# jc-bao/gym-formation

Hardware: AMD Instinct MI355X
Metric: env-steps/sec (higher is better)
Workload: dtype f32

## Files before the change

gym-formation_amd/csrc/fg_common.hpp:

```cpp
#ifndef FG_COMMON_HPP_
#define FG_COMMON_HPP_


#include <hip/hip_runtime.h>
#include <stdint.h>
#include <stdio.h>
#include <string.h>

#include "formation_hip.h"


namespace fg {

#define FG_DEV __device__ __forceinline__
constexpr int FG_PRODUCER_PRIO = 2;
typedef float f32x4 __attribute__((ext_vector_type(4)));
typedef float f32x2 __attribute__((ext_vector_type(2)));

#ifndef FG_F64
#define FG_F64 0
#endif
#if FG_F64
typedef double real;
typedef double2 real2;
// ... 11 lines not shown
FG_DEV float rabs(float a) { return fabsf(a); }
FG_DEV float rsqrt_(float a) { return sqrtf(a); }
FG_DEV float rfma(float a, float b, float c) { return __builtin_fmaf(a, b, c); }
FG_DEV float hw_sqrt(float a) { return __builtin_amdgcn_sqrtf(a); }
FG_DEV float hw_rcp(float a) { return __builtin_amdgcn_rcpf(a); }
FG_DEV float hw_log(float a) { return __logf(a); }
FG_DEV float hw_exp(float a) { return __expf(a); }
FG_DEV double rmin(double a, double b) { return fmin(a, b); }
FG_DEV double rmax(double a, double b) { return fmax(a, b); }
FG_DEV double rabs(double a) { return fabs(a); }
FG_DEV double rsqrt_(double a) { return sqrt(a); }
FG_DEV double rfma(double a, double b, double c) { return __builtin_fma(a, b, c); }
FG_DEV double hw_sqrt(double a) { return sqrt(a); }
FG_DEV double hw_rcp(double a) { return 1.0 / a; }
FG_DEV double hw_log(double a) { return log(a); }
FG_DEV double hw_exp(double a) { return exp(a); }

#if FG_F64
struct KWall {
    int32_t vertical, soft;
    double axis_pos, end0, end1, width;
};
struct KParams {
    double dt, damping, contact_force, contact_margin, sensitivity, mass, dist_min, collide_thresh;
    int32_t world_length, auto_reset;
    uint64_t seed, rng_offset;
    double accel, max_speed, u_noise;
    int32_t num_walls;
    KWall walls[FG_MAX_WALLS];
    int32_t obs_env_pitch, env_index_base;
    const uint64_t* rng_offset_dev;
    const double* agent_props;
    const double* comm_state;
    int32_t obs_placed, reserved0;
};
#else
typedef FgParams KParams;
typedef FgWall KWall;
#endif
FG_DEV uint64_t rng_base(const KParams& p) { return p.rng_offset + (p.rng_offset_dev ? *p.rng_offset_dev : 0ull); }

__host__ __device__ constexpr int npad(int n) { return (n + 3) & ~3; }
__host__ __device__ constexpr int env_block_floats(int n) { return 10 * n + 6 * npad(n); }
FG_DEV real2* env_tables(real2* smem, int ee, int n) {
    return reinterpret_cast<real2*>(reinterpret_cast<real*>(smem) + ee * env_block_floats(n));
}
FG_DEV const real2* env_tables(const real2* smem, int ee, int n) {
    return reinterpret_cast<const real2*>(reinterpret_cast<const real*>(smem) + ee * env_block_floats(n));
}
__host__ __device__ constexpr int step_lds_bytes(int n, int e, bool opts) {
    return (e * env_block_floats(n) + 72 + (opts ? 3 * npad(n) + 2 * e * n : 0)) * (int)sizeof(real);
}
constexpr real FAR_AWAY = 1.0e18f;

constexpr int FG_POLICY_MAX_LEVELS = 10;
struct FgPolicyLevels {
    int per, L;
    float inv_per;
    float inv_sub[FG_POLICY_MAX_LEVELS];
};

struct Args {
    KParams p;
    int B, N, K, obs_every;
    real inv_n;
    int do_phys, do_post;
    int groups;
// ... 167 lines not shown
```

gym-formation_amd/csrc/fg_obs_writers.hpp:

```cpp
#ifndef FG_OBS_WRITERS_HPP_
#define FG_OBS_WRITERS_HPP_

#include "fg_common.hpp"

namespace fg {

template <class V2> FG_DEV V2 lds_if(bool c, const V2* __restrict__ p, int idx_if_true) {
    V2 t = p[c ? idx_if_true : 0];
    t.x = c ? t.x : 0.0f; t.y = c ? t.y : 0.0f;
    return t;
}

constexpr bool FG_ROWS_MERGED = true;
template <int NC, int NW, int E, int PACE = 0>
FG_DEV void write_obs_rows(const real2* __restrict__ tables0, int env_stride, int w,
                           real2* __restrict__ out_env0, size_t env_units, int El, int parts,
                           int wg_part = 0, int wg_parts = 1, bool pace_on = true) {
    constexpr int N = NC;
    constexpr int WPE = (E >= NW) ? 1 : NW / E;
    constexpr int ESTEP = (E >= NW) ? NW : 1;
    static_assert((E >= NW) ? (E % NW == 0) : (NW % E == 0), "waves and envs must tile");
    const int lane = threadIdx.x & 63;
    const int row0 = (E >= NW) ? 0 : w % WPE;
    constexpr unsigned ROWU = 3u * N;
// ... 85 lines not shown
            for (int c = 0; c < CD; ++c) {
                const int u = lane + 64 * c;
                Pm[c] = lds_if(u >= 1 && u < N, AA, u - 1);
                Pu[c] = lds_if(u >= 1 && u < N, AA, u);
            }
#pragma unroll
            for (int c = 0; c < CS; ++c) sv[c] = lds_if(lane + 64 * c < 2 * N, AA, N + lane + 64 * c);
            const int nshare = WPE * wg_parts, share = wg_part * WPE + row0;
            const int PER = (N + nshare - 1) / nshare;
            const int r_end = min(N, (share + 1) * PER);
#pragma unroll 2
            for (int r = share * PER; r < r_end; ++r) {
                const real2 xp = AA[r];
                const real2 x0 = AA[(lane == 0 ? 4 * N : 0) + r];
                real2* __restrict__ orow = out + (unsigned)r * ROWU;
#pragma unroll
                for (int c = 0; c < CD; ++c) {
                    const int u = lane + 64 * c;
                    const real2 x = (c == 0) ? x0 : xp;
                    const real2 cc = (u - 1 >= r) ? Pu[c] : Pm[c];
                    if ((parts & 1) && u < N) orow[u] = make_real2(cc.x - x.x, cc.y - x.y);
                }
#pragma unroll
                for (int c = 0; c < CS; ++c)
                    if ((parts & 2) && lane + 64 * c < 2 * N) orow[N + lane + 64 * c] = sv[c];
                if (PACE > 0 && pace_on) __builtin_amdgcn_s_sleep(PACE);
            }
        }
    }
}

template <int NC, int RT> constexpr int tile_units() { return (3 * NC * RT + 16 + 2 + 1) & ~1; }

template <int NC, int NW, int E, int RT, bool STREAM>
FG_DEV void write_obs_tiled(const float2* __restrict__ tables0, int env_stride, int w, float2* __restrict__ tiles,
                            float2* __restrict__ out_env0, size_t unit0, size_t env_units, int El) {
    constexpr int N = NC;
    constexpr int WPE = (E >= NW) ? 1 : NW / E;
    static_assert((E >= NW) ? (E % NW == 0) : (NW % E == 0), "waves and envs must tile");
    static_assert(N <= 32 && N % RT == 0, "tiled writer: N <= 32, RT divides N");
    constexpr unsigned ROWU = 3u * N, TU = ROWU * RT;
    constexpr int TILES_ENV = N / RT;
    constexpr int MY_TILES = (TILES_ENV + WPE - 1) / WPE;
    const int lane = threadIdx.x & 63;
    float2* tile0 = tiles + w * 2 * tile_units<NC, RT>();
    constexpr int RW = 64 / N;
    const int rsub = lane / N, u = lane - rsub * N;
    const bool act = rsub < RW;
    const int xoff = (u == 0) ? 4 * N : 0;
    constexpr int RS = 64 / (2 * N);
    const int ssub = lane / (2 * N), sidx = lane - ssub * 2 * N;
    const int e_first = (E >= NW) ? w : w / WPE, e_step = (E >= NW) ? NW : E;
    const int t_first = (E >= NW) ? 0 : w % WPE;
    const int n_env = (El > e_first) ? (El - e_first + e_step - 1) / e_step : 0;
    const int total = n_env * MY_TILES;

    constexpr unsigned ENVU = ROWU * N;
    const unsigned pad = (unsigned)(env_units - ENVU);
    static_assert(!STREAM || (E >= NW && NC >= 16), "streaming form: waves own whole envs, rows of >= 16 units");
    const bool own = STREAM && ((unit0 & 15) == 0) && (pad == 0 || (pad < 16 && (env_units & 15) == 0));
    auto head_units = [&](int ee) -> unsigned {
        return (own && pad == 0) ? (16u - (unsigned)(((size_t)ee * env_units) & 15)) & 15u : 0u;
    };
    auto extra_units = [&](int ee) -> unsigned {
        if (!own) return 0u;
        if (pad) return pad;
        return (ee + 1 < El) ? head_units(ee + 1) : 0u;
    };

// ... 17 lines not shown
        }
        const unsigned par = (unsigned)((unit0 + (size_t)ee * env_units + (size_t)r0 * ROWU) & 1);
        float2* img = tile0 + (t & 1) * tile_units<NC, RT>() + par;
#pragma unroll
        for (int rb = 0; rb < RT; rb += RW) {
            const int rl = rb + rsub;
            if (act && rl < RT) {
                const int r = r0 + rl;
                const float2 x = AA[xoff + r];
                const float2 c = (u - 1 >= r) ? Pu : Pm;
                img[(unsigned)rl * ROWU + (unsigned)u] = make_float2(c.x - x.x, c.y - x.y);
            }
        }
#pragma unroll
        for (int rb = 0; rb < RT; rb += RS) {
            const int rl = rb + ssub;
            if (ssub < RS && rl < RT) img[(unsigned)rl * ROWU + (unsigned)(N + sidx)] = sv;
        }
        if (STREAM && r0 + RT == N) {
            const unsigned x = extra_units(ee);
            if ((unsigned)lane < x) {
                float2 val = make_float2(0.f, 0.f);
                if (pad == 0) {
                    static_assert(ROWU >= 16, "the line remainder must stay inside row 0 of the next env");
                    const float2* __restrict__ A1 = tables0 + (size_t)(ee + 1) * env_stride;
                    const float2 a = A1[lane == 0 ? 3 * N : lane], b = A1[0];
                    const bool rel = lane >= 1 && lane < N;
                    val = make_float2(a.x - (rel ? b.x : 0.f), a.y - (rel ? b.y : 0.f));
                }
                img[TU + (unsigned)lane] = val;
            }
        }
    };
    auto stream = [&](int t) {
        int ee, r0; locate(t, ee, r0);
        if (r0 >= N) return;
        const unsigned par = (unsigned)((unit0 + (size_t)ee * env_units + (size_t)r0 * ROWU) & 1);
        const float2* img = tile0 + (t & 1) * tile_units<NC, RT>() + par;
        float2* __restrict__ out = out_env0 + (size_t)ee * env_units + (size_t)r0 * ROWU;
        if constexpr (!STREAM) {
            if (par && lane == 0) out[0] = img[0];
            constexpr unsigned NPMAX = TU >> 1;
            const unsigned npair = (TU - par) >> 1;
            const f32x4* src4 = reinterpret_cast<const f32x4*>(img + par);
            f32x4* __restrict__ dst4 = reinterpret_cast<f32x4*>(out + par);
#pragma unroll
            for (unsigned q0 = 0; q0 < NPMAX; q0 += 64) {
                const unsigned q = q0 + lane;
                if (q < npair) dst4[q] = src4[q];
            }
            if (((TU - par) & 1u) && lane == 63) out[TU - 1] = img[TU - 1];
        } else {
            const unsigned s = (r0 == 0) ? head_units(ee) : 0u;
            const unsigned end = TU + ((r0 + RT == N) ? extra_units(ee) : 0u);
            const unsigned p2 = (par + s) & 1u;
            if (p2 && lane == 0) out[s] = img[s];
            constexpr unsigned NPMAX = (TU + 16) >> 1;
            const unsigned npair = (end - s - p2) >> 1;
            const f32x4* src4 = reinterpret_cast<const f32x4*>(img + s + p2);
            f32x4* __restrict__ dst4 = reinterpret_cast<f32x4*>(out + s + p2);
            constexpr unsigned NFULL = ((TU - 16) >> 1) / 64;
#pragma unroll
            for (unsigned c = 0; c < NFULL; ++c) {
                const f32x4 v = src4[c * 64 + lane];
                asm volatile("s_waitcnt lgkmcnt(0)" ::: "memory");
                dst4[c * 64 + lane] = v;
                asm volatile("" ::: "memory");
                __builtin_amdgcn_s_sleep(1);
            }
#pragma unroll
            for (unsigned q0 = NFULL * 64; q0 < NPMAX; q0 += 64) {
                const unsigned q = q0 + lane;
                if (q < npair) dst4[q] = src4[q];
            }
            if (((end - s - p2) & 1u) && lane == 63) out[end - 1] = img[end - 1];
        }
    };
    if (total > 0) compose(0);
    for (int t = 0; t < total; ++t) {
        if (t + 1 < total) compose(t + 1);
        stream(t);
    }
}

constexpr int FG_WR_GATHER = 64;
template <int NC> constexpr int gather_passes() { return (3 * NC * NC / 2 + 2 + 63) / 64; }
template <int NC> constexpr int gather_lut_units() { return 2 * gather_passes<NC>() * 64 * 2; }

template <int NC>
FG_DEV void build_gather_lut(uint4* __restrict__ lut, int t, int nthreads) {
    constexpr int N = NC, ROWU = 3 * N, TU = ROWU * N, P = gather_passes<NC>() * 64;
    static_assert(N >= 2 && 5 * N < 65536, "gather writer: table offsets are 16-bit, the table's zeros are the 0 operand");
    auto operands = [&](int unit, unsigned& a, unsigned& b) {
        const int r = unit / ROWU, u = unit - r * ROWU;
        if (u == 0) { a = N; b = 4 * N + r; }
        else if (u < N) { a = (u - 1 >= r) ? u : u - 1; b = r; }
        else { a = u; b = N; }
    };
    for (int e = t; e < 2 * P; e += nthreads) {
        const int par = e / P, q = e - par * P;
        const int npair = (TU - par) >> 1;
        const bool tail = ((TU - par) & 1) != 0;
        int unit = -1, kind = 0;
        if (q < npair) { unit = 2 * q + par; kind = 2; }
        else if (par && q == npair) { unit = 0; kind = 1; }
        else if (tail && q == npair + par) { unit = TU - 1; kind = 1; }
        unsigned a0 = N, b0 = N, a1 = N, b1 = N;
        if (kind >= 1) operands(unit, a0, b0);
        if (kind == 2) operands(unit + 1, a1, b1);
        lut[e] = make_uint4(a0 | (b0 << 16), a1 | (b1 << 16), (unsigned)(unit < 0 ? 0 : unit) | ((unsigned)kind << 16), 0u);
    }
}

template <int NC> struct GatherEntries {
// ... 203 lines not shown
```

gym-formation_amd/csrc/fg_rollout_kernels.hpp:

```cpp
#ifndef FG_ROLLOUT_KERNELS_HPP_
#define FG_ROLLOUT_KERNELS_HPP_

#include "fg_common.hpp"
#include "fg_pair_loops.hpp"
#include "fg_obs_writers.hpp"
#include "fg_policy_kernels.hpp"

namespace fg {

__host__ __device__ constexpr int roll_block_floats(int n) { return 20 * n + 6 * npad(n); }
template <int NC, int WR, int NWW, int E> constexpr int roll_writer_units() {
    if constexpr (WR == 0) return 0;
    else if constexpr (roll_writer_obs16(WR)) return 2 * NWW * obs16_tile_words<NC, NWW, E>() / 2;
    else if constexpr (WR == FG_WR_GATHER)
        return gather_lut_units<NC>() > E * 3 * NC * NC / 2 ? gather_lut_units<NC>() : E * 3 * NC * NC / 2;
    else return 2 * NWW * tile_units<NC, WR - 1>();
}

template <int NC, int TW, int E, int WR, int PER> constexpr int roll_lds_base_bytes() {
    return E * roll_block_floats(NC) * (int)sizeof(real) + roll_writer_units<NC, WR, TW / 64, E>() * (int)sizeof(float2) +
           (PER > 0 ? E * policy_block_units(NC) * (int)sizeof(float2) : 0);
}
template <int NC, int E> constexpr int roll_rew_floats() { return 2 * 3 * E * NC; }
template <int NC, int TW, int E, int WR, int PER> constexpr bool roll_rew_in_lds() {
// ... 203 lines not shown
                }
            }
            int slot = k;
            bool want_obs = a.obs != nullptr;
            if (a.obs_every > 1) { want_obs = want_obs && ((k + 1) % a.obs_every == 0); slot = k / a.obs_every; }
            if (want_obs) {
                const size_t unit0 = ((size_t)slot * a.B + b0) * (size_t)a.obs_pitch;
                const size_t env_units = (size_t)a.obs_pitch;
                const real2* tables0 = reinterpret_cast<const real2*>(smemf) + (k & 1) * 5 * N;
                if constexpr (WR == 0)
                    write_obs_rows<NC, NWW, E>(tables0, roll_block_floats(N) / 2, (tid - TP) >> 6,
                                               reinterpret_cast<real2*>(a.obs) + unit0, env_units, El, 3);
                else if constexpr (WR == FG_WR_GATHER) {
                  if (use_span)
                    Span::write(span_lut, tables0, (tid - TP) >> 6, reinterpret_cast<real2*>(a.obs) + unit0);
                  else {
                    GatherEntries<(WR == FG_WR_GATHER ? NC : 2)> gather_entries;
                    write_obs_gather<NC, NWW, E>(tables0, roll_block_floats(N) / 2, (tid - TP) >> 6,
                                                 reinterpret_cast<const uint4*>(smemf + E * roll_block_floats(N)),
                                                 reinterpret_cast<real2*>(a.obs) + unit0, unit0, env_units, El, gather_entries);
                  }
                }
#if !FG_F64
                else if constexpr (roll_writer_obs16(WR)) {
                    static_assert((E * roll_block_floats(NC)) % 4 == 0, "the 16-bit writer's tiles start on a 16-byte boundary");
                    write_obs16<NC, NWW, E, WR>(tables0, roll_block_floats(N) / 2, (tid - TP) >> 6,
                                                reinterpret_cast<uint32_t*>(smemf + E * roll_block_floats(N)),
                                                reinterpret_cast<uint32_t*>(a.obs) + unit0, unit0, El);
                }
#endif
                else
                    write_obs_tiled<NC, NWW, E, WR - 1, STREAM>(tables0, roll_block_floats(N) / 2, (tid - TP) >> 6,
                                                                reinterpret_cast<real2*>(smemf + E * roll_block_floats(N)),
                                                                reinterpret_cast<real2*>(a.obs) + unit0, unit0, env_units, El);
            }
        }
        __syncthreads();
    };
    if constexpr (ACT4) {
        for (int k = 0; k < a.K; k += 4) {
            if (producer && k + 4 < a.K) load_batch(nxt, k + 4);
            pipeline_step(k, cur[1], u_odd);
            if (k + 1 < a.K) pipeline_step(k + 1, cur[2], u_odd);
            if (k + 2 < a.K) pipeline_step(k + 2, cur[3], u_odd);
            if (k + 3 < a.K) pipeline_step(k + 3, nxt[0], u_odd);
#pragma unroll
            for (int t = 0; t < 4; ++t) cur[t] = nxt[t];
        }
    } else {
        for (int k = 0; k < a.K; k += 2) {
            pipeline_step(k, u_odd, u_even);
            if (k + 1 < a.K) pipeline_step(k + 1, u_even, u_odd);
        }
    }
    if (valid) {
        int is = i, bs = b;
        asm volatile("" : "+v"(is), "+v"(bs));
        const size_t so = (size_t)bs * N + is;
        a.px[so] = p.x; a.py[so] = p.y; a.vx[so] = v.x; a.vy[so] = v.y;
    }
    if (a.step && env_ok && i == 0) a.step[b] = t_step;
}

template <int NC, int A, int E, int TW, int PER = 0, bool BATCHES = false>
__global__ __launch_bounds__(E * 64 + TW) void rollout_kernel_wide(const Args a) {
    constexpr bool POLICY = PER > 0;
    static_assert(!(BATCHES && POLICY), "the batch-pipelined single step takes its actions from the caller");
// ... 300 lines not shown
```

gym-formation_amd/formation_gym/_native.py:

```python
import ctypes
import os
import subprocess

_HERE = os.path.dirname(os.path.abspath(__file__))
_PKG_ROOT = os.path.dirname(_HERE)
LIB_PATH = os.path.join(_PKG_ROOT, "lib", "libformation_hip.so")
BUILD_SCRIPT = os.path.join(_PKG_ROOT, "csrc", "build.sh")

ABI_VERSION = 8
MAX_WALLS = 4
AGENT_PROPS = 8
AGENT_IMMOVABLE, AGENT_NO_COLLIDE, AGENT_GHOST, AGENT_SCRIPTED = 1, 2, 4, 8

FG_OK = 0
FG_ERR_BAD_ARG = -1
FG_ERR_UNSUPPORTED_N = -2
FG_ERR_ALIGNMENT = -3
FG_ERR_HIP = -4


class FgWall(ctypes.Structure):
    _fields_ = [("vertical", ctypes.c_int32), ("axis_pos", ctypes.c_float), ("end0", ctypes.c_float),
                ("end1", ctypes.c_float), ("width", ctypes.c_float), ("soft", ctypes.c_int32)]


class FgParams(ctypes.Structure):
    _fields_ = [
        ("dt", ctypes.c_float),
        ("damping", ctypes.c_float),
        ("contact_force", ctypes.c_float),
        ("contact_margin", ctypes.c_float),
        ("sensitivity", ctypes.c_float),
        ("mass", ctypes.c_float),
        ("dist_min", ctypes.c_float),
        ("collide_thresh", ctypes.c_float),
        ("world_length", ctypes.c_int32),
        ("auto_reset", ctypes.c_int32),
        ("seed", ctypes.c_uint64),
        ("rng_offset", ctypes.c_uint64),
        ("accel", ctypes.c_float),
        ("max_speed", ctypes.c_float),
        ("u_noise", ctypes.c_float),
        ("num_walls", ctypes.c_int32),
        ("walls", FgWall * 4),
        ("obs_env_pitch", ctypes.c_int32),
        ("env_index_base", ctypes.c_int32),
        ("rng_offset_dev", ctypes.c_void_p),
        ("agent_props", ctypes.c_void_p),
        ("comm_state", ctypes.c_void_p),
        ("obs_placed", ctypes.c_int32),
        ("reserved0", ctypes.c_int32),
    ]


FG_SCN_BASIC, FG_SCN_PARTIAL, FG_SCN_RANGE, FG_SCN_OBSTACLE = 1, 2, 3, 4
FG_ACT_ONEHOT5, FG_ACT_INDEX, FG_ACT_ARGMAX = 1, 2, 3
FG_OBS_F16, FG_OBS_BF16 = 1, 2


def obs_format(dtype):
    import torch
    if dtype is None:
        return 0
    if dtype == torch.float16:
        return FG_OBS_F16
    if dtype == torch.bfloat16:
        return FG_OBS_BF16
    raise ValueError("obs_dtype must be None, torch.float16 or torch.bfloat16; got %r" % (dtype,))


class FgScenario(ctypes.Structure):
    _fields_ = [
        ("kind", ctypes.c_int32),
        ("num_landmarks", ctypes.c_int32),
        ("num_obstacles", ctypes.c_int32),
        ("num_obs", ctypes.c_int32),
        ("obs_range", ctypes.c_float),
        ("obstacle_size", ctypes.c_float),
        ("obstacle_vx", ctypes.c_float),
        ("obstacle_vy", ctypes.c_float),
        ("obstacle_floor", ctypes.c_float),
        ("penalty", ctypes.c_float),
        ("variant", ctypes.c_int32),
        ("reserved", ctypes.c_int32),
# ... 265 lines not shown
```

gym-formation_amd/formation_gym/environment.py:

```python
import numbers

import numpy as np
import torch

from . import _native, actor_rollout, spaces

cam_range = 2


class MultiAgentEnv(object):
    metadata = {'render.modes': ['human', 'rgb_array']}

    def __init__(self, world, reset_callback=None, reward_callback=None,
                 observation_callback=None, info_callback=None,
                 done_callback=None, post_step_callback=None,
                 shared_viewer=True, discrete_action=False):
        self.world = world
        self.world_length = self.world.world_length
        self.current_step = 0
        self.agents = self.world.policy_agents
        self.num_agents = len(world.policy_agents)
        self.reset_callback = reset_callback
        self.reward_callback = reward_callback
        self.observation_callback = observation_callback
        self.info_callback = info_callback
        self.done_callback = done_callback
        self.post_step_callback = post_step_callback
        self.num_envs = world.num_envs
        self.scenario = world.scenario
        if self.scenario is None:
            raise ValueError("world.scenario is not set: make_world() must attach the Scenario "
                             "that owns the batched kernels")
        self.discrete_action_space = bool(discrete_action)
        self.discrete_action_input = False
        self.force_discrete_action = bool(getattr(world, 'discrete_action', False))
        self.shared_reward = world.collaborative if hasattr(world, 'collaborative') else False
        self.time = 0
        self.auto_reset = False
# ... 137 lines not shown

    def _rollout_out(self, want, out, K, obs_every, policy, obs_dtype=None):
        placed = out is None and self.default_placed and obs_dtype is None
        if placed:
            out = self._default_out(K, obs_every, policy)
        elif out is None or out is False:
            return {k: self._fresh_out(k, want[k], obs_dtype) for k in want}, False
        own_buffers = True
        for k in ("log_prob", "rnn_states", "idx"):
            if k not in want:
                continue
            if placed and tuple(getattr(out.get(k), "shape", ())) != want[k]:
                out[k] = self._fresh_out(k, want[k])
            elif k not in out:
                out, own_buffers = dict(out, **{k: self._fresh_out(k, want[k])}), False
            elif k == "rnn_states":
                self._state_tensor("out['rnn_states']", out[k], want[k], None)
            elif k == "idx" and (not torch.is_tensor(out[k]) or out[k].dtype != torch.int32):
                raise ValueError("out['idx'] must be an int32 tensor of shape %s" % (want[k],))
        return out, own_buffers

    def _fresh_out(self, k, shape, obs_dtype=None):
        if k == "done":
            return torch.zeros(shape, dtype=torch.uint8, device=self._act.device)
        if k == "idx":
            return torch.empty(shape, dtype=torch.int32, device=self._act.device)
        return torch.empty(shape, dtype=(obs_dtype or torch.float32) if k == "obs" else torch.float32, device=self._act.device)

    def _run_rollout(self, lead_key, want, out, own_buffers, K, obs_every, obs_dtype, bind, unbound, args, extra=()):
        key = None
        if own_buffers and bind is not None and want.keys() <= out.keys():
            key = lead_key + (tuple([out[k].data_ptr() for k in want]), tuple(out["obs"].stride()), obs_every,
                              self.auto_reset, _native.current_stream_fast(self.world.device), self.world.params_signature(),
                              getattr(self.scenario, "_seed", 0), obs_dtype)
        launch = self._roll_launchers.get(key) if key is not None else None
        off = self._launch_rng_offset()
        if launch is None:
            for k, shp in want.items():
                if k not in out or tuple(out[k].shape) != shp or not (out[k].is_contiguous() or k == "obs"):
                    raise ValueError("out[%r] must be a contiguous tensor of shape %s" % (k, shp))
            self._check_obs_dtype(out, obs_dtype)
            kw = dict(extra, obs_every=obs_every, auto_reset=self.auto_reset)
            if obs_dtype is not None:
                kw["obs_format"] = _native.obs_format(obs_dtype)
            if key is not None or unbound is None:
                launch = bind(self.world, *args, out, **kw)
            if key is not None:
                if len(self._roll_launchers) >= 8:
                    self._roll_launchers.clear()
                self._roll_launchers[key] = launch
        if launch is not None:
            launch(off)
            self.scenario._cache = None
        else:
            unbound(self.world, *args, out, rng_offset=off, **kw)
        self._advance_rng(K)
        self.current_step += K
        self.world.world_step += K

    def _rollout_result(self, out, info=(), rew=None):
        if rew is None:
            rew = out["reward"] if self.shared_reward else out["indiv"]
        info = dict(info, individual_reward=out["indiv"])
        return out["obs"], rew.unsqueeze(-1), out["done"].view(torch.bool), info

    def _rollout_by_steps(self, action_seq, out, obs_every):
        K, obs_every = self._check_steps(len(action_seq), obs_every)
        dev = self._act.device
        want = self._rollout_shapes(K, obs_every)
        if out is None or out is False:
            out = self._rollout_out(want, False, K, obs_every, False)[0]
        for k, shp in want.items():
            if k not in out or tuple(out[k].shape) != shp:
                raise ValueError("out[%r] must be a tensor of shape %s" % (k, shp))
        first = None if self.shared_reward else torch.empty(want["reward"], dtype=torch.float32, device=dev)
        for k in range(K):
            act = action_seq[k]
            if torch.is_tensor(act) and (act.dtype != torch.float32 or act.device != dev) and not self._action_mode():
                act = act.to(device=dev, dtype=torch.float32)
            o, r, d, info = self.step(act if torch.is_tensor(act) else torch.as_tensor(act, device=dev))
            out["reward"][k].copy_(self._out["reward"]); out["indiv"][k].copy_(self._out["indiv"])
            out["done"][k].copy_(self._out["done"])
            if first is not None:
                first[k].copy_(r[..., 0])
            if (k + 1) % obs_every == 0:
                out["obs"][k // obs_every].copy_(o)
        return self._rollout_result(out, rew=first)

    def _step_loop(self, K, obs_every, act_fn, after_step=None):
        res = {k: [] for k in ("obs", "rew", "done", "indiv", "act")}
        obs = self._out["obs"]
        for k in range(K):
            act = act_fn(obs, k)
            res["act"].append(act.clone() if torch.is_tensor(act) else torch.as_tensor(act, device=self._act.device))
            obs, r, d, info = self.step(act)
            if (k + 1) % obs_every == 0:
                res["obs"].append(obs.clone())
            res["rew"].append(r.clone()); res["done"].append(d.clone()); res["indiv"].append(info["individual_reward"].clone())
            if after_step is not None:
                after_step(d)
        return (torch.stack(res["obs"]) if res["obs"] else obs.new_empty((0,) + tuple(obs.shape)), torch.stack(res["rew"]),
                torch.stack(res["done"]), {"individual_reward": torch.stack(res["indiv"]), "actions": torch.stack(res["act"])})

    def rollout_policy(self, K, num_agents_per_layer=3, out=None, obs_every=1, obs_dtype=None):
        roll = getattr(self.scenario, "rollout_policy_batch", None)
        if roll is None:
            raise NotImplementedError("%s has no built-in controller" % type(self.scenario).__name__)
        if self._action_mode():
# ... 322 lines not shown
                raise RuntimeError("rollout(out=None) inside a placement probe")
            while len(self._auto_out) >= 4:
                self._auto_out.pop(next(iter(self._auto_out)))
            self._roll_launchers.clear()
            out = self.alloc_rollout_buffers(K, obs_every=obs_every, policy=policy, escalate=False)
        self._auto_out[key] = out
        return out

    def _snapshot(self):
        w, sc = self.world, self.scenario
        dev = {k: getattr(w, k).clone() for k in ("pos_x", "pos_y", "vel_x", "vel_y", "step_count", "landmark_pos",
                                                  "obstacle_pos", "obstacle_vel")
               if torch.is_tensor(getattr(w, k, None))}
        scn = {k: getattr(sc, k).clone() for k in ("ideal_shape", "ideal_vel") if torch.is_tensor(getattr(sc, k, None))}
        ctr = None if w.rng_counter is None else w.rng_counter.clone()
        own = sc.snapshot_state() if hasattr(sc, "snapshot_state") else None
        return dev, scn, ctr, (self._rng_offset, self.current_step, w.world_step), own

    def _restore(self, snap):
        dev, scn, ctr, host, own = snap
        w, sc = self.world, self.scenario
        if own is not None:
            sc.restore_state(own)
        for k, v in dev.items():
            getattr(w, k).copy_(v)
        for k, v in scn.items():
            getattr(sc, k).copy_(v)
        if ctr is not None:
            w.rng_counter.copy_(ctr)
        self._rng_offset, self.current_step, w.world_step = host
        sc._cache = None

    def alloc_rollout_buffers(self, K, obs_every=1, obs_env_pitch=0, policy=False, candidates=8, mem_fraction=0.5,
                              max_arena_bytes=None, escalate=True):
        from . import placement
        K, obs_every = int(K), int(obs_every)
        B, N = self.num_envs, self.num_agents
        D = self._out["obs"].shape[-1]
        dev = self._act.device
        f = dict(dtype=torch.float32, device=dev)
        slots = K // obs_every
        pitch = int(obs_env_pitch) if obs_env_pitch else N * D
        if pitch < N * D or pitch % 2:
            raise ValueError("obs_env_pitch must be 0 or an even number of floats >= %d" % (N * D))
        small = dict(reward=torch.empty((K, B, N), **f), indiv=torch.empty((K, B, N), **f),
                     done=torch.zeros((K, B, N), dtype=torch.uint8, device=dev))
        if policy:
            small["act"] = torch.empty((K, B, N, 2), **f)

        def shaped(flat):
            return flat.view(slots, B, pitch)[:, :, :N * D].view(slots, B, N, D)

        def alloc():
            return shaped(torch.empty(slots * B * pitch, **f))

        nbytes = slots * B * pitch * 4
        if slots == 0 or nbytes < placement.MIN_PROBE_BYTES or candidates < 2:
            self.placement = {"tried": 1, "probed": False}
            return dict(small, obs=alloc())
        snap = self._snapshot()
        closed = policy and getattr(self.scenario, "rollout_policy_batch", None) is not None
        acts = None if closed else torch.zeros((K, B, N, 2), **f)

        per_layer = self._policy_per_layer() if closed else 0

        def time_fn(obs):
            out = dict(small, obs=obs)
            if closed:
                self.rollout_policy(K, per_layer, out=out, obs_every=obs_every)
            else:
                self.rollout(acts, out=out, obs_every=obs_every)
            self._roll_launchers.clear()

        arena = None
        self._placing = True
        modes = (self.discrete_action_input, self.discrete_action_space, self.force_discrete_action)
        self.discrete_action_input = self.discrete_action_space = self.force_discrete_action = False
        try:
            placed = placement.probe_arena(slots * B * pitch, lambda flat: time_fn(shaped(flat)), dev, trials=candidates,
                                           mem_fraction=mem_fraction, max_arena_bytes=max_arena_bytes, escalate=escalate)
            if placed is not None:
                flat, report, arena = placed
                obs = shaped(flat)
            else:
                obs, report = placement.probe_allocation(alloc, time_fn, nbytes, dev, candidates=candidates, mem_fraction=mem_fraction)
        finally:
            self._placing = False
            self.discrete_action_input, self.discrete_action_space, self.force_discrete_action = modes
            self._roll_launchers.clear()
            torch.cuda.empty_cache()
            self._restore(snap)
        report["buffer_MB"] = round(nbytes / 1e6, 1)
        if report.get("probed") and D == 6 * N:
            alg = _native.step_hd_bytes(N) * B * K
            report["kept_GBps"] = round(alg / (report["kept_ms"] * 1e-3) / 1e9, 1)
            report["worst_GBps"] = round(alg / (report["worst_ms"] * 1e-3) / 1e9, 1)
        self.placement = report
        return dict(small, obs=obs)

    def _policy_per_layer(self):
        N = self.num_agents
        for per in (3, 2, 4, 5, 6, 7, 8):
            n = per
            while n < N:
                n *= per
            if n == N:
                return per
        raise ValueError("the built-in controller needs N = per^L agents with 2 <= per <= 8, got %d" % N)

    def place_step_buffers(self, candidates=8, mem_fraction=0.5):
        from . import placement
        B, N = self.num_envs, self.num_agents
        obs_dim = self._out["obs"].shape[-1]
        n_obs, n_bn = B * N * obs_dim, B * N
        nflat = n_obs + 2 * n_bn + (n_bn + 3) // 4
        dev = self._act.device
        if n_obs * 4 < placement.MIN_PROBE_BYTES or candidates < 2:
            self.placement = {"tried": 1, "probed": False}
            return self.placement
        extra = {k: v for k, v in self._out.items() if k not in ("obs", "reward", "indiv", "done")}

        def views(flat):
            return dict(extra, obs=flat[:n_obs].view(B, N, obs_dim), reward=flat[n_obs:n_obs + n_bn].view(B, N),
                        indiv=flat[n_obs + n_bn:n_obs + 2 * n_bn].view(B, N),
                        done=flat[n_obs + 2 * n_bn:].view(torch.uint8)[:n_bn].view(B, N))

        snap = self._snapshot()
        old_flat, self._flat, self._out = self._flat, None, None
        del old_flat
        torch.cuda.empty_cache()
        act = torch.zeros_like(self._act)
# ... 216 lines not shown
```

gym-formation_amd/formation_gym/envs/formation_hd_env.py:

```python
import ctypes

import numpy as np
import torch

from formation_gym import _native, placement
from formation_gym.core import World, Agent, Landmark
from formation_gym.scenario import BaseScenario


class _Plan(object):

    def __init__(self, lib, handle, keep):
        self.lib, self.handle, self.keep = lib, handle, keep

    def __del__(self):
        try:
            if self.handle:
                self.lib.fg_plan_destroy(self.handle)
                self.handle = None
        except Exception:
            pass


class Scenario(BaseScenario):
    def make_world(self, num_agents=3, episode_length=100, num_envs=1, device=None):
        world = World(num_envs=num_envs, device=device)
        world.world_length = episode_length
        world.dim_c = 2
        world.collaborative = True
        self.num_agents = num_agents
        world.agents = [Agent() for _ in range(num_agents)]
        for i, agent in enumerate(world.agents):
            agent.name = 'agent %d' % i
            agent.collide = True
            agent.silent = True
            agent.size = 0.03
        world.landmarks = [Landmark() for _ in range(num_agents)]
        for i, landmark in enumerate(world.landmarks):
            landmark.name = 'landmarks %d' % i
            landmark.collide = False
            landmark.movable = False
            landmark.size = 0.01
        world.allocate()
        world.scenario = self
        B, N = world.num_envs, num_agents
        f = dict(dtype=torch.float32, device=world.device)
        self.ideal_shape = torch.zeros((B, N, 2), **f)
        self.ideal_vel = torch.zeros((B, 2), **f)
        self._rngs = None
        self._seed = 1
        self._cache = None
        self.reset_world(world)
        return world

    def seed(self, seed=None):
        self._seed = 1 if seed is None else int(seed)
        self._rngs = None
# ... 27 lines not shown
        world.landmark_pos.copy_(torch.as_tensor(lm, dtype=torch.float32))
        if env_mask is None:
            world.step_count.zero_()
        else:
            m = torch.as_tensor(np.asarray(env_mask, dtype=bool), device=world.device)
            world.step_count.masked_fill_(m, 0)
        self._cache = None

    def set_formation(self, world, ideal_shape=None, ideal_vel=None):
        if ideal_shape is not None:
            self.ideal_shape.copy_(torch.as_tensor(np.array(ideal_shape), dtype=torch.float32))
        if ideal_vel is not None:
            self.ideal_vel.copy_(torch.as_tensor(np.array(ideal_vel), dtype=torch.float32))
        self._cache = None

    def obs_dim(self, world):
        return 6 * len(world.agents)

    def params(self, world, auto_reset=False, rng_offset=0, obs=None, scripted_ok=False):
        a0 = world.agents[0]
        p = world.native_params(collide_thresh=(a0.size + a0.size) / 2,
                                auto_reset=auto_reset, seed=self._seed, rng_offset=rng_offset, scripted_ok=scripted_ok)
        p.obs_env_pitch = self.obs_env_pitch(obs, len(world.agents))
        p.env_index_base = int(getattr(self, "env_base", 0))
        if world.any_non_silent():
            if world.dim_c != 2:
                raise NotImplementedError("formation_hd_env's observation has a communication block of dim_c = 2 (:40, :48-51); "
                                          "World.step / update_agent_state take any dim_c")
            comm = world.ensure_comm()[0]
            p.comm_state = comm.data_ptr()
            p._pinned += (comm,)
        if obs is not None and obs.numel() and placement.is_placed(obs.data_ptr()):
            p.obs_placed = 1
        return p

    @staticmethod
    def obs_env_pitch(obs, N):
        if obs is None or obs.numel() == 0 or obs.is_contiguous():
            return 0
        D = 6 * N
        ok = obs.dim() in (3, 4) and obs.stride(-1) == 1 and obs.stride(-2) == D and obs.shape[-2:] == (N, D)
        B = obs.shape[-3] if ok else 0
        slots = obs.shape[0] if ok and obs.dim() == 4 else 1
        if ok and B > 1:
            pitch = obs.stride(-3)
            if slots > 1:
                ok = obs.stride(0) == B * pitch
        elif ok and slots > 1:
            pitch = obs.stride(0)
        else:
            pitch = N * D
        if not ok or pitch < N * D or pitch % 2:
            raise ValueError("observation tensor must be [.., B, N, 6N] with dense rows and a uniform even env pitch "
                             ">= 6 N^2 floats; got shape %s strides %s" % (tuple(obs.shape), tuple(obs.stride())))
        if pitch == N * D:
            return 0
        return int(pitch)

    def _state_ptrs(self, world, act):
        return (world.pos_x.data_ptr(), world.pos_y.data_ptr(), world.vel_x.data_ptr(), world.vel_y.data_ptr(),
                act.data_ptr(), self.ideal_shape.data_ptr(), self.ideal_vel.data_ptr(), world.step_count.data_ptr())

    @staticmethod
    def _out_ptrs(out):
        return (_native.ptr(out.get("obs")), out["reward"].data_ptr(), _native.ptr(out.get("indiv")),
                _native.ptr(out.get("done")))

# ... 290 lines not shown
```

gym-formation_amd/formation_gym/placement.py:

```python
import ctypes

import torch

from . import _native

MIN_PROBE_BYTES = 256 << 20


def _time_launch(time_fn, buf, stream, reps):
    time_fn(buf)
    ev = [torch.cuda.Event(enable_timing=True) for _ in range(reps + 1)]
    ev[0].record(stream)
    for r in range(reps):
        time_fn(buf)
        ev[r + 1].record(stream)
    stream.synchronize()
    t = sorted(ev[r].elapsed_time(ev[r + 1]) for r in range(reps))
    return t[len(t) // 2]


def probe_allocation(alloc, time_fn, nbytes, device, candidates=8, mem_fraction=0.6, reps=3, min_bytes=MIN_PROBE_BYTES,
                     good_enough=0.90, min_tried=4):
    device = torch.device(device)
    free = torch.cuda.mem_get_info(device)[0] if device.type == "cuda" else 0
# ... 13 lines not shown
        if len(ms) >= min_tried and min(ms) <= good_enough * max(ms):
            break
    best = min(range(len(ms)), key=lambda i: ms[i])
    keep = held[best]
    del held, buf
    torch.cuda.empty_cache()
    return keep, {"method": "allocations", "tried": len(ms), "max_candidates": m, "ms": [round(x, 4) for x in ms], "kept": best,
                  "probed": True, "kept_ms": round(ms[best], 4), "worst_ms": round(max(ms), 4),
                  "worst_over_kept": round(max(ms) / ms[best], 4)}


class _LaunchError(Exception):
    """Wraps an exception raised by the caller's own launch (`time_fn`) inside a probe, so that it is not mistaken for an
    arena / mapping failure (which falls back to whole allocations with a warning)."""


_live_arenas = []


def is_placed(address):
    address = int(address)
    alive = []
    hit = False
    for ref in _live_arenas:
        arena = ref()
        if arena is None or arena._handle is None:
            continue
        alive.append(ref)
        lo, hi = arena.kept_range
        if lo <= address < hi:
            hit = True
    _live_arenas[:] = alive
    return hit


class _Raw(object):

    def __init__(self, ptr, nfloats, owner=None):
        self.__cuda_array_interface__ = {"shape": (int(nfloats),), "typestr": "<f4", "data": (int(ptr), False), "version": 2}
        self.owner = owner


class Arena(object):

    def __init__(self, nbytes, device, chunk_bytes=0):
        self.device = torch.device(device)
        index = self.device.index if self.device.index is not None else torch.cuda.current_device()
        handle, chunk, count = ctypes.c_void_p(), ctypes.c_uint64(), ctypes.c_uint32()
        _native.check(_native.load().fg_arena_create(int(index), int(nbytes), int(chunk_bytes), ctypes.byref(handle),
                                                     ctypes.byref(chunk), ctypes.byref(count)))
        self._handle, self.chunk, self.chunks = handle, int(chunk.value), int(count.value)
        self.kept_range = (0, 0)
        import weakref
        _live_arenas.append(weakref.ref(self))

    def floats(self, address, nfloats):
        return torch.as_tensor(_Raw(int(address), nfloats, self), device=self.device)

    def map(self, chunk_index):
        arr = (ctypes.c_uint32 * len(chunk_index))(*[int(c) for c in chunk_index])
        base = ctypes.c_void_p()
        _native.check(_native.load().fg_arena_map(self._handle, arr, len(chunk_index), ctypes.byref(base)))
        return int(base.value)

    def unmap(self, base):
        _native.check(_native.load().fg_arena_unmap(self._handle, ctypes.c_void_p(int(base))))
# ... 248 lines not shown
```

include/formation_hip.h:

```cpp
#ifndef FORMATION_HIP_H_
#define FORMATION_HIP_H_

#include <stdint.h>

#ifdef __cplusplus
extern "C" {
#endif

#define FG_ABI_VERSION 8
#define FG_MAX_AGENTS 1024
#define FG_MAX_WALLS 4

typedef enum FgStatus {
    FG_OK = 0,
    FG_ERR_BAD_ARG = -1,
    FG_ERR_UNSUPPORTED_N = -2,
    FG_ERR_ALIGNMENT = -3,
    FG_ERR_HIP = -4
} FgStatus;

typedef struct FgWall {
    int32_t vertical;
    float axis_pos;
    float end0, end1;
    float width;
    int32_t soft;
} FgWall;

typedef struct FgParams {
    float dt;
    float damping;
    float contact_force;
    float contact_margin;
    float sensitivity;
    float mass;
    float dist_min;
    float collide_thresh;
    int32_t world_length;
    int32_t auto_reset;
    uint64_t seed;
    uint64_t rng_offset;
    float accel;
    float max_speed;
    float u_noise;
    int32_t num_walls;
    FgWall walls[FG_MAX_WALLS];
    int32_t obs_env_pitch;
    int32_t env_index_base;
    const uint64_t* rng_offset_dev;
    const float* agent_props;
    const float* comm_state;
    int32_t obs_placed;
    int32_t reserved0;
} FgParams;
#define FG_AGENT_PROPS 8
#define FG_AGENT_IMMOVABLE 1
#define FG_AGENT_NO_COLLIDE 2
#define FG_AGENT_GHOST 4
#define FG_AGENT_SCRIPTED 8

typedef enum FgScenarioKind {
    FG_SCN_BASIC = 1, FG_SCN_PARTIAL = 2, FG_SCN_RANGE = 3, FG_SCN_OBSTACLE = 4
} FgScenarioKind;

typedef struct FgScenario {
    int32_t kind;
    int32_t num_landmarks;
    int32_t num_obstacles;
    int32_t num_obs;
    float obs_range;
    float obstacle_size;
    float obstacle_vx;
    float obstacle_vy;
    float obstacle_floor;
    float penalty;
    int32_t variant;
    int32_t reserved;
} FgScenario;

int fg_arena_create(int device, uint64_t bytes, uint64_t chunk_bytes, void** arena, uint64_t* chunk_out, uint32_t* chunks_out);
int fg_arena_map(void* arena, const uint32_t* chunk_index, uint32_t count, void** base);
int fg_arena_unmap(void* arena, void* base);
int fg_arena_keep_window(void* arena, void* base, uint32_t first, uint32_t count, void** new_base);
int fg_arena_trim(void* arena);
uint64_t fg_arena_retired_address_bytes(void);
int fg_arena_destroy(void* arena);
// ... 300 lines not shown
```

Measured before the change: 345.9 million.

## Skip storing always-zero observation blocks into pre-zeroed rollout buffers

Rollout obs buffers are zeroed once and registered in a Python-side primed registry. A new kernel flag tells the tiled obs writer to skip 128-byte store groups that fall entirely inside the structurally zero part of each obs row. The goal is to cut global write traffic in a store-bound writer. In exchange it adds per-lane predicate arithmetic and a host-side tracking layer for address, extent and generation, and it depends on nothing else overwriting the buffer between calls. Allocation keeps the mode only if a quick A/B timing favours it.

```diff
diff --git a/gym-formation_amd/csrc/fg_common.hpp b/gym-formation_amd/csrc/fg_common.hpp
--- a/gym-formation_amd/csrc/fg_common.hpp
+++ b/gym-formation_amd/csrc/fg_common.hpp
@@ -67,7 +67,7 @@
     const uint64_t* rng_offset_dev;
     const double* agent_props;
     const double* comm_state;
-    int32_t obs_placed, reserved0;
+    int32_t obs_placed, obs_zero_primed;
 };
 #else
 typedef FgParams KParams;
diff --git a/gym-formation_amd/csrc/fg_obs_writers.hpp b/gym-formation_amd/csrc/fg_obs_writers.hpp
--- a/gym-formation_amd/csrc/fg_obs_writers.hpp
+++ b/gym-formation_amd/csrc/fg_obs_writers.hpp
@@ -141,9 +141,29 @@
 
 template <int NC, int RT> constexpr int tile_units() { return (3 * NC * RT + 16 + 2 + 1) & ~1; }
 
+constexpr unsigned FG_ZERO_SKIP_BYTES = 128;
+template <bool B> struct ZeroPrimed { static constexpr bool value = B; };
+template <int NC> constexpr bool zero_skip_fits() { return NC >= 16 && NC - 1 >= (int)(FG_ZERO_SKIP_BYTES / 8); }
+template <int NC> FG_DEV unsigned zero_skip_m0(bool primed, const void* row0, unsigned u0) {
+    constexpr unsigned GU = FG_ZERO_SKIP_BYTES / 8, ROWU = 3u * NC;
+    static_assert(ROWU > GU && 128u % GU == 0, "a group in front of row 0 lies in the row before; 1 KiB is whole groups");
+    if constexpr (!zero_skip_fits<NC>()) return 0u;
+    if (!primed) return 0u;
+    const unsigned ph = ((unsigned)(uintptr_t)row0 >> 3) & (GU - 1u);
+    const unsigned g0 = ((u0 + ph) & ~(GU - 1u)) - ph + ROWU;
+    return g0 % ROWU;
+}
+template <int NC> FG_DEV bool zero_skip_at(bool primed, unsigned m0, unsigned c) {
+    constexpr unsigned GU = FG_ZERO_SKIP_BYTES / 8, ROWU = 3u * NC;
+    if constexpr (!zero_skip_fits<NC>()) return false;
+    unsigned m = m0 + (c * 128u) % ROWU;
+    m = min(m, m - ROWU);
+    return primed && m - (unsigned)NC <= (unsigned)(NC - 1) - GU;
+}
+
 template <int NC, int NW, int E, int RT, bool STREAM>
 FG_DEV void write_obs_tiled(const float2* __restrict__ tables0, int env_stride, int w, float2* __restrict__ tiles,
-                            float2* __restrict__ out_env0, size_t unit0, size_t env_units, int El) {
+                            float2* __restrict__ out_env0, size_t unit0, size_t env_units, int El, bool primed = false) {
     constexpr int N = NC;
     constexpr int WPE = (E >= NW) ? 1 : NW / E;
     static_assert((E >= NW) ? (E % NW == 0) : (NW % E == 0), "waves and envs must tile");
@@ -227,7 +247,8 @@
             }
         }
     };
-    auto stream = [&](int t) {
+    auto stream = [&](int t, auto PR) {
+        constexpr bool primed = decltype(PR)::value;
         int ee, r0; locate(t, ee, r0);
         if (r0 >= N) return;
         const unsigned par = (unsigned)((unit0 + (size_t)ee * env_units + (size_t)r0 * ROWU) & 1);
@@ -239,10 +260,11 @@
             const unsigned npair = (TU - par) >> 1;
             const f32x4* src4 = reinterpret_cast<const f32x4*>(img + par);
             f32x4* __restrict__ dst4 = reinterpret_cast<f32x4*>(out + par);
+            const unsigned m0 = zero_skip_m0<NC>(primed, out, par + 2u * lane);
 #pragma unroll
             for (unsigned q0 = 0; q0 < NPMAX; q0 += 64) {
                 const unsigned q = q0 + lane;
-                if (q < npair) dst4[q] = src4[q];
+                if (q < npair && !zero_skip_at<NC>(primed, m0, q0 / 64)) dst4[q] = src4[q];
             }
             if (((TU - par) & 1u) && lane == 63) out[TU - 1] = img[TU - 1];
         } else {
@@ -254,19 +276,21 @@
             const unsigned npair = (end - s - p2) >> 1;
             const f32x4* src4 = reinterpret_cast<const f32x4*>(img + s + p2);
             f32x4* __restrict__ dst4 = reinterpret_cast<f32x4*>(out + s + p2);
+            const unsigned m0 = zero_skip_m0<NC>(primed, out, s + p2 + 2u * lane);
             constexpr unsigned NFULL = ((TU - 16) >> 1) / 64;
 #pragma unroll
             for (unsigned c = 0; c < NFULL; ++c) {
                 const f32x4 v = src4[c * 64 + lane];
+                const bool skip = zero_skip_at<NC>(primed, m0, c);
                 asm volatile("s_waitcnt lgkmcnt(0)" ::: "memory");
-                dst4[c * 64 + lane] = v;
+                if (!skip) dst4[c * 64 + lane] = v;
                 asm volatile("" ::: "memory");
                 __builtin_amdgcn_s_sleep(1);
             }
 #pragma unroll
             for (unsigned q0 = NFULL * 64; q0 < NPMAX; q0 += 64) {
                 const unsigned q = q0 + lane;
-                if (q < npair) dst4[q] = src4[q];
+                if (q < npair && !zero_skip_at<NC>(primed, m0, q0 / 64)) dst4[q] = src4[q];
             }
             if (((end - s - p2) & 1u) && lane == 63) out[end - 1] = img[end - 1];
         }
@@ -274,7 +298,8 @@
     if (total > 0) compose(0);
     for (int t = 0; t < total; ++t) {
         if (t + 1 < total) compose(t + 1);
-        stream(t);
+        if (primed) stream(t, ZeroPrimed<true>{});
+        else stream(t, ZeroPrimed<false>{});
     }
 }
 
diff --git a/gym-formation_amd/csrc/fg_rollout_kernels.hpp b/gym-formation_amd/csrc/fg_rollout_kernels.hpp
--- a/gym-formation_amd/csrc/fg_rollout_kernels.hpp
+++ b/gym-formation_amd/csrc/fg_rollout_kernels.hpp
@@ -259,7 +259,8 @@
                 else
                     write_obs_tiled<NC, NWW, E, WR - 1, STREAM>(tables0, roll_block_floats(N) / 2, (tid - TP) >> 6,
                                                                 reinterpret_cast<real2*>(smemf + E * roll_block_floats(N)),
-                                                                reinterpret_cast<real2*>(a.obs) + unit0, unit0, env_units, El);
+                                                                reinterpret_cast<real2*>(a.obs) + unit0, unit0, env_units, El,
+                                                                a.p.obs_zero_primed != 0);
             }
         }
         __syncthreads();
diff --git a/gym-formation_amd/formation_gym/_native.py b/gym-formation_amd/formation_gym/_native.py
--- a/gym-formation_amd/formation_gym/_native.py
+++ b/gym-formation_amd/formation_gym/_native.py
@@ -49,7 +49,7 @@
         ("agent_props", ctypes.c_void_p),
         ("comm_state", ctypes.c_void_p),
         ("obs_placed", ctypes.c_int32),
-        ("reserved0", ctypes.c_int32),
+        ("obs_zero_primed", ctypes.c_int32),
     ]
 
 
diff --git a/gym-formation_amd/formation_gym/environment.py b/gym-formation_amd/formation_gym/environment.py
--- a/gym-formation_amd/formation_gym/environment.py
+++ b/gym-formation_amd/formation_gym/environment.py
@@ -3,7 +3,7 @@
 import numpy as np
 import torch
 
-from . import _native, actor_rollout, spaces
+from . import _native, actor_rollout, placement, spaces
 
 cam_range = 2
 
@@ -207,7 +207,7 @@
         if own_buffers and bind is not None and want.keys() <= out.keys():
             key = lead_key + (tuple([out[k].data_ptr() for k in want]), tuple(out["obs"].stride()), obs_every,
                               self.auto_reset, _native.current_stream_fast(self.world.device), self.world.params_signature(),
-                              getattr(self.scenario, "_seed", 0), obs_dtype)
+                              getattr(self.scenario, "_seed", 0), obs_dtype, placement._primed_gen[0])
         launch = self._roll_launchers.get(key) if key is not None else None
         off = self._launch_rng_offset()
         if launch is None:
@@ -249,6 +249,8 @@
             if k not in out or tuple(out[k].shape) != shp:
                 raise ValueError("out[%r] must be a tensor of shape %s" % (k, shp))
         first = None if self.shared_reward else torch.empty(want["reward"], dtype=torch.float32, device=dev)
+        if torch.is_tensor(out["obs"]) and out["obs"].numel():
+            placement.drop_primed(out["obs"].data_ptr(), out["obs"].numel() * out["obs"].element_size())
         for k in range(K):
             act = action_seq[k]
             if torch.is_tensor(act) and (act.dtype != torch.float32 or act.device != dev) and not self._action_mode():
@@ -637,8 +639,7 @@
         sc._cache = None
 
     def alloc_rollout_buffers(self, K, obs_every=1, obs_env_pitch=0, policy=False, candidates=8, mem_fraction=0.5,
-                              max_arena_bytes=None, escalate=True):
-        from . import placement
+                              max_arena_bytes=None, escalate=True, primed=True):
         K, obs_every = int(K), int(obs_every)
         B, N = self.num_envs, self.num_agents
         D = self._out["obs"].shape[-1]
@@ -660,7 +661,16 @@
             return shaped(torch.empty(slots * B * pitch, **f))
 
         nbytes = slots * B * pitch * 4
-        if slots == 0 or nbytes < placement.MIN_PROBE_BYTES or candidates < 2:
+        primed = bool(primed) and slots > 0 and D == 6 * N and getattr(self.scenario, "obs_zero_block", False)
+
+        def prime(obs, keeper=None):
+            if primed:
+                obs.zero_()
+                placement.register_primed(obs if keeper is None else keeper, obs.data_ptr(), nbytes, N, B, pitch)
+            return obs
+
+        probe = not (slots == 0 or nbytes < placement.MIN_PROBE_BYTES or candidates < 2)
+        if not probe and not primed:
             self.placement = {"tried": 1, "probed": False}
             return dict(small, obs=alloc())
         snap = self._snapshot()
@@ -669,7 +679,9 @@
 
         per_layer = self._policy_per_layer() if closed else 0
 
-        def time_fn(obs):
+        def time_fn(obs, keeper=None, auto=True):
+            if auto and primed and not placement.is_primed(obs.data_ptr(), nbytes, N, B, pitch):
+                prime(obs, keeper)
             out = dict(small, obs=obs)
             if closed:
                 self.rollout_policy(K, per_layer, out=out, obs_every=obs_every)
@@ -682,26 +694,50 @@
         modes = (self.discrete_action_input, self.discrete_action_space, self.force_discrete_action)
         self.discrete_action_input = self.discrete_action_space = self.force_discrete_action = False
         try:
-            placed = placement.probe_arena(slots * B * pitch, lambda flat: time_fn(shaped(flat)), dev, trials=candidates,
-                                           mem_fraction=mem_fraction, max_arena_bytes=max_arena_bytes, escalate=escalate)
-            if placed is not None:
+            placed = None if not probe else \
+                placement.probe_arena(slots * B * pitch, lambda flat: time_fn(shaped(flat), flat), dev, trials=candidates,
+                                      mem_fraction=mem_fraction, max_arena_bytes=max_arena_bytes, escalate=escalate)
+            if not probe:
+                obs, report = alloc(), {"tried": 1, "probed": False}
+            elif placed is not None:
                 flat, report, arena = placed
                 obs = shaped(flat)
             else:
                 obs, report = placement.probe_allocation(alloc, time_fn, nbytes, dev, candidates=candidates, mem_fraction=mem_fraction)
+            placement.drop_primed(obs.data_ptr(), nbytes)
+            if primed:
+                stream = torch.cuda.current_stream(dev)
+                prime(obs)
+                t_on = placement._time_launch(lambda o: time_fn(o, auto=False), obs, stream, 5)
+                placement.drop_primed(obs.data_ptr(), nbytes)
+                t_off = placement._time_launch(lambda o: time_fn(o, auto=False), obs, stream, 5)
+                primed = t_on <= 0.98 * t_off
+                report["zero_primed"] = {"kept": primed, "flagged_ms": round(t_on, 4), "unflagged_ms": round(t_off, 4)}
         finally:
             self._placing = False
             self.discrete_action_input, self.discrete_action_space, self.force_discrete_action = modes
             self._roll_launchers.clear()
             torch.cuda.empty_cache()
             self._restore(snap)
-        report["buffer_MB"] = round(nbytes / 1e6, 1)
+        if probe:
+            report["buffer_MB"] = round(nbytes / 1e6, 1)
         if report.get("probed") and D == 6 * N:
             alg = _native.step_hd_bytes(N) * B * K
             report["kept_GBps"] = round(alg / (report["kept_ms"] * 1e-3) / 1e9, 1)
             report["worst_GBps"] = round(alg / (report["worst_ms"] * 1e-3) / 1e9, 1)
         self.placement = report
-        return dict(small, obs=obs)
+        return dict(small, obs=prime(obs))
+
+    def prime_rollout_buffers(self, out):
+        obs = out["obs"]
+        B, N = self.num_envs, self.num_agents
+        if not getattr(self.scenario, "obs_zero_block", False) or obs.dtype != torch.float32 or obs.dim() != 4 \
+                or tuple(obs.shape[1:]) != (B, N, 6 * N):
+            raise ValueError("prime_rollout_buffers: out['obs'] must be a float32 [slots, %d, %d, %d] tensor of formation_hd_env" % (B, N, 6 * N))
+        pitch = self.scenario.obs_env_pitch(obs, N) or 6 * N * N
+        obs.zero_()
+        placement.register_primed(obs, obs.data_ptr(), ((obs.shape[0] * B - 1) * pitch + 6 * N * N) * 4, N, B, pitch)
+        return out
 
     def _policy_per_layer(self):
         N = self.num_agents
diff --git a/gym-formation_amd/formation_gym/envs/formation_hd_env.py b/gym-formation_amd/formation_gym/envs/formation_hd_env.py
--- a/gym-formation_amd/formation_gym/envs/formation_hd_env.py
+++ b/gym-formation_amd/formation_gym/envs/formation_hd_env.py
@@ -23,6 +23,8 @@
 
 
 class Scenario(BaseScenario):
+    obs_zero_block = True
+
     def make_world(self, num_agents=3, episode_length=100, num_envs=1, device=None):
         world = World(num_envs=num_envs, device=device)
         world.world_length = episode_length
@@ -116,7 +118,21 @@
             p._pinned += (comm,)
         if obs is not None and obs.numel() and placement.is_placed(obs.data_ptr()):
             p.obs_placed = 1
+        if obs is None or not placement.near_primed(obs):
+            pass
+        elif p.comm_state or obs.dtype != torch.float32:
+            placement.drop_primed(obs.data_ptr(), obs.numel() * obs.element_size())
+        else:
+            N = len(world.agents)
+            pitch = p.obs_env_pitch or 6 * N * N
+            if placement.is_primed(obs.data_ptr(), self._obs_extent(obs, p.obs_env_pitch, N), N, world.num_envs, pitch, launch=True):
+                p.obs_zero_primed = 1
         return p
+
+    @staticmethod
+    def _obs_extent(obs, env_pitch, N):
+        blocks = obs.numel() // (6 * N * N)
+        return ((blocks - 1) * (env_pitch or 6 * N * N) + 6 * N * N) * obs.element_size()
 
     @staticmethod
     def obs_env_pitch(obs, N):
diff --git a/gym-formation_amd/formation_gym/placement.py b/gym-formation_amd/formation_gym/placement.py
--- a/gym-formation_amd/formation_gym/placement.py
+++ b/gym-formation_amd/formation_gym/placement.py
@@ -69,6 +69,66 @@
             hit = True
     _live_arenas[:] = alive
     return hit
+
+
+_primed = []
+_primed_gen = [0]
+
+
+def primed_generation():
+    return _primed_gen[0]
+
+
+def _primed_alive():
+    alive = [e for e in _primed if e[0]() is not None]
+    if len(alive) != len(_primed):
+        _primed[:] = alive
+        _primed_gen[0] += 1
+    return _primed
+
+
+def register_primed(keeper, address, nbytes, N, B, pitch):
+    import weakref
+    drop_primed(address, nbytes)
+    _primed.append([weakref.ref(keeper), int(address), int(nbytes), int(N), int(B), int(pitch)])
+    _primed_gen[0] += 1
+
+
+def drop_primed(address, nbytes=1):
+    lo, hi = int(address), int(address) + max(1, int(nbytes))
+    keep = [e for e in _primed_alive() if e[1] + e[2] <= lo or hi <= e[1]]
+    hit = len(keep) != len(_primed)
+    if hit:
+        _primed[:] = keep
+        _primed_gen[0] += 1
+    return hit
+
+
+def near_primed(obs):
+    if not _primed:
+        return False
+    n = obs.numel()
+    if not n:
+        return False
+    lo = obs.data_ptr()
+    hi = lo + 2 * n * obs.element_size()
+    for e in _primed:
+        if e[1] < hi and lo < e[1] + e[2]:
+            return True
+    return False
+
+
+def is_primed(address, nbytes, N, B, pitch, launch=False):
+    address, end = int(address), int(address) + int(nbytes)
+    for ref, base, size, n, b, p in list(_primed_alive()):
+        if end <= base or base + size <= address:
+            continue
+        if base <= address and end <= base + size and (n, b, p) == (int(N), int(B), int(pitch)) \
+                and (address - base) % (4 * b * p) == 0:
+            return True
+        if launch:
+            drop_primed(base, size)
+    return False
 
 
 class _Raw(object):
diff --git a/include/formation_hip.h b/include/formation_hip.h
--- a/include/formation_hip.h
+++ b/include/formation_hip.h
@@ -51,7 +51,7 @@
     const float* agent_props;
     const float* comm_state;
     int32_t obs_placed;
-    int32_t reserved0;
+    int32_t obs_zero_primed;
 } FgParams;
 #define FG_AGENT_PROPS 8
 #define FG_AGENT_IMMOVABLE 1
diff --git a/profiles/r06_zero_skip/holes.hip b/profiles/r06_zero_skip/holes.hip
--- /dev/null
+++ b/profiles/r06_zero_skip/holes.hip
@@ -0,0 +1,105 @@
+#include <hip/hip_runtime.h>
+#include <cstdio>
+#include <cstdlib>
+typedef float f32x4 __attribute__((ext_vector_type(4)));
+typedef float f32x2 __attribute__((ext_vector_type(2)));
+#define CHECK(x) do { hipError_t e_ = (x); if (e_ != hipSuccess) { printf("HIP error %s at %d\n", hipGetErrorString(e_), __LINE__); exit(1); } } while (0)
+
+constexpr int N = 27, ROWB = 3 * N * 8, ENVB = ROWB * N;
+constexpr int Z0 = N * 8, Z1 = (2 * N - 1) * 8;
+constexpr int K = 20, B = 4096, G = 256, E = 16, NW = 8;
+constexpr unsigned SPAN = (unsigned)E * ENVB;
+
+__device__ __forceinline__ bool in_zero(unsigned o) {
+    const unsigned off = o % ROWB;
+    return off >= Z0 && off < Z1;
+}
+template <unsigned GB> __device__ __forceinline__ bool group_in_zero(unsigned a) {
+    const unsigned g0 = a & ~(GB - 1), es = (a / ENVB) * ENVB;
+    if (g0 < es || g0 + GB > es + ENVB) return false;
+    const unsigned off = (g0 - es) % ROWB;
+    return off >= Z0 && off + GB <= Z1;
+}
+
+template <int ARM> __global__ __launch_bounds__(NW * 64) void k_holes(char* out) {
+    const int w = threadIdx.x >> 6, lane = threadIdx.x & 63;
+    const f32x4 v = {1.f, 2.f, 3.f, 4.f};
+    for (int k = 0; k < K; ++k) {
+        char* slab = out + (size_t)k * B * ENVB;
+        const unsigned span0 = blockIdx.x * SPAN;
+        for (int e = w; e < E; e += NW) {
+            const unsigned s = span0 + (((unsigned)e * ENVB + 127u) & ~127u);
+            const unsigned end = span0 + (e + 1 == E ? SPAN : (((unsigned)(e + 1) * ENVB + 127u) & ~127u));
+            for (unsigned a0 = s; a0 < end; a0 += 1024u) {
+                const unsigned a = a0 + 16u * lane;
+                if (a < end) {
+                    if (ARM == 0) {
+                        *reinterpret_cast<f32x4*>(slab + a) = v;
+                    } else if (ARM == 1) {
+                        if (!group_in_zero<64>(a)) *reinterpret_cast<f32x4*>(slab + a) = v;
+                    } else if (ARM == 2) {
+                        if (!group_in_zero<128>(a)) *reinterpret_cast<f32x4*>(slab + a) = v;
+                    } else {
+                        const unsigned o = a % ENVB;
+                        const bool z0 = in_zero(o), z1 = in_zero(o + 8 < ENVB ? o + 8 : 0);
+                        if (!z0 && !z1) *reinterpret_cast<f32x4*>(slab + a) = v;
+                        else if (!z0) *reinterpret_cast<f32x2*>(slab + a) = f32x2{1.f, 2.f};
+                        else if (!z1) *reinterpret_cast<f32x2*>(slab + a + 8) = f32x2{3.f, 4.f};
+                    }
+                }
+                asm volatile("" ::: "memory");
+                __builtin_amdgcn_s_sleep(1);
+            }
+        }
+    }
+}
+
+template <int ARM> float run(char* buf, hipEvent_t e0, hipEvent_t e1, int reps) {
+    for (int i = 0; i < 3; ++i) hipLaunchKernelGGL(k_holes<ARM>, dim3(G), dim3(NW * 64), 0, 0, buf);
+    CHECK(hipEventRecord(e0));
+    for (int i = 0; i < reps; ++i) hipLaunchKernelGGL(k_holes<ARM>, dim3(G), dim3(NW * 64), 0, 0, buf);
+    CHECK(hipEventRecord(e1));
+    CHECK(hipEventSynchronize(e1));
+    float ms; CHECK(hipEventElapsedTime(&ms, e0, e1));
+    return ms / reps * 1e3f;
+}
+
+int main() {
+    const size_t bytes = (size_t)K * B * ENVB;
+    char* buf;
+    CHECK(hipMalloc(&buf, bytes + 4096));
+    CHECK(hipMemset(buf, 0, bytes + 4096));
+    hipEvent_t e0, e1;
+    CHECK(hipEventCreate(&e0)); CHECK(hipEventCreate(&e1));
+    double stored[4] = {0, 0, 0, 0};
+    for (unsigned a = 0; a < (unsigned)B * ENVB; a += 16) {
+        auto giz = [&](unsigned GB) {
+            const unsigned g0 = a & ~(GB - 1), es = (a / ENVB) * ENVB;
+            if (g0 < es || g0 + GB > es + ENVB) return false;
+            const unsigned off = (g0 - es) % ROWB;
+            return off >= (unsigned)Z0 && off + GB <= (unsigned)Z1;
+        };
+        auto iz = [&](unsigned x) { const unsigned off = (x % ENVB) % ROWB; return off >= (unsigned)Z0 && off < (unsigned)Z1; };
+        stored[0] += 16;
+        stored[1] += giz(64) ? 0 : 16;
+        stored[2] += giz(128) ? 0 : 16;
+        stored[3] += (iz(a) ? 0 : 8) + (iz(a + 8) ? 0 : 8);
+    }
+    const char* names[4] = {"full", "skip64", "skip128", "exact"};
+    for (int i = 0; i < 4; ++i) printf("%-8s stores %.1f %% of the bytes\n", names[i], 100.0 * stored[i] / stored[0]);
+    const int PASSES = 6, REP = 20;
+    float lo[4] = {1e30f, 1e30f, 1e30f, 1e30f}, hi[4] = {0, 0, 0, 0};
+    for (int pass = 0; pass < PASSES; ++pass)
+        for (int arm = 0; arm < 4; ++arm) {
+            const float us = arm == 0 ? run<0>(buf, e0, e1, REP) : arm == 1 ? run<1>(buf, e0, e1, REP)
+                           : arm == 2 ? run<2>(buf, e0, e1, REP) : run<3>(buf, e0, e1, REP);
+            lo[arm] = us < lo[arm] ? us : lo[arm]; hi[arm] = us > hi[arm] ? us : hi[arm];
+            printf("pass %d  %-8s  %.1f us/launch  %.2f us/slab  %.2f TB/s (bytes a consumer sees)\n", pass, names[arm], us, us / K,
+                   (double)bytes / (us * 1e-6) / 1e12);
+        }
+    for (int arm = 0; arm < 4; ++arm)
+        printf("%-8s  %.1f - %.1f us/launch%s\n", names[arm], lo[arm], hi[arm],
+               arm == 0 ? "" : hi[arm] < lo[0] ? "  every pass faster than every pass of full" : "  NOT clearly faster than full");
+    CHECK(hipFree(buf));
+    return 0;
+}
```

New measurement: 372.2 million (median of 6 runs). 7.6% higher.
